# Kiripiro/leaffliction

Hardware: AMD Instinct MI355X
Metric: 224x224 images/sec train (higher is better)
Workload: dtype f32; 1 GPU; leaf_cnn base train step (configs[1]: img 224, batch 256/GPU, fp32, 8 classes, AdamW+clipnorm+EMA, in-model augmentation); per_gpu_batch=256, global_batch=256, img_size=224, parallelism=dp1

## Files before the change

### include/leafhip.h

```cpp
#ifndef LEAFHIP_H
#define LEAFHIP_H

#include <stddef.h>
#include <stdint.h>

#ifdef __cplusplus
extern "C" {
#endif

#define LF_OK 0
#define LF_ERR_INVALID (-1)
#define LF_ERR_LAUNCH (-2)
#define LF_ERR_WORKSPACE (-3)

#define LF_VERSION 100

typedef void* lf_stream_t;

int lf_version(void);
const char* lf_last_error(void);

int lf_copy_rows(void* dst, size_t dst_pitch, const void* src, size_t src_pitch, size_t width, size_t rows, int to_host,
                 lf_stream_t stream);

// ... 211 lines not shown
                                 uint16_t* pooled, int n, int c, int h, int w, lf_stream_t stream);
int lf_block_tail_bwd_bf16(const uint16_t* dp, const uint8_t* route, const uint16_t* y,
                           const float* a_scale, const float* a_shift, const float* drop, uint16_t* dr,
                           float* ds, float* plane_sums, const uint16_t* sc_y, float* sc_sums, int n,
                           int c, int h, int w, lf_stream_t stream);
int lf_bcast_planes_bf16(const float* v, uint16_t* out, int planes, int hw, float scale,
                         lf_stream_t stream);
int lf_cast_f32_bf16(const float* in, uint16_t* out, size_t count, lf_stream_t stream);
int lf_cast_bf16_f32(const uint16_t* in, float* out, size_t count, lf_stream_t stream);

int lf_conv2d_variant(int h, int wd, int cout, int ksize);
int lf_conv2d_wgrad_variant(int n, int cin, int h, int wd, int cout, int ksize);

int lf_conv2d_plan(int n, int cin, int h, int wd, int cout, int ksize, int* out);
int lf_conv2d_wgrad_plan(int n, int cin, int h, int wd, int cout, int ksize, int* out);
int lf_conv2d_bf16_plan(int n, int cin, int h, int w, int cout, int ksize, int x_bf16, int y_bf16, int entry,
                        int accumulate, int mask, int* out);
int lf_conv2d_wgrad_bf16_plan(int n, int cin, int h, int w, int cout, int ksize, int* out);

long long lf_conv2d_stats_tiles(int n, int cin, int h, int w, int cout, int ksize);
int lf_conv2d_stats_f32(const float* x, const float* w, float* y, int n, int cin, int h, int wd,
                        int cout, int ksize, const float* in_scale, const float* in_shift,
                        int in_relu, const float* pivot, float* tile_part, size_t tile_part_bytes,
                        lf_stream_t stream, const float* wino_u);

int lf_conv2d_bnbwd_f32(const float* x, const float* w, float* y, int n, int cin, int h, int wd,
                        int cout, int ksize, int accumulate, const float* mask_y,
                        const float* mask_scale, const float* mask_shift, int mask_relu,
                        float* tile_part, size_t tile_part_bytes, lf_stream_t stream, const float* wino_u);

// ... 98 lines not shown
```

### leaffliction_amd/_lib.py

```python
from __future__ import annotations

import ctypes as C
import os
from pathlib import Path

_LIB = None

LIB_PATH = Path(__file__).resolve().parent / "libleafhip.so"

c_void_p, c_int, c_size_t, c_u64, c_float, c_double = (
    C.c_void_p, C.c_int, C.c_size_t, C.c_uint64, C.c_float, C.c_double)
P = c_void_p

SIGNATURES = {
    "lf_version": [],
    "lf_last_error": [],
    "lf_pack_hwc_u8_to_nchw_f32": [P, P, c_int, c_int, c_int, P, P, P],
    "lf_hist_u8": [P, P, c_int, c_int, c_int, P],
    "lf_autocontrast_lut": [P, P, P, c_int, P],
    "lf_lut_apply_u8": [P, P, P, c_int, c_int, c_int, P],
    "lf_gather_rows_u8": [P, P, P, c_int, c_size_t, P],
    "lf_flip_u8": [P, P, P, c_int, c_int, c_int, P],
    "lf_noise_wrap_add_u8": [P, P, P, c_size_t, P],
    "lf_add_wrap_u8": [P, P, P, c_size_t, P],
# ... 61 lines not shown
    "lf_conv2d_bf16_train": [P, c_int, P, P, c_int, c_int, c_int, c_int, c_int, c_int, P, P, c_int, c_int, P,
                             c_size_t, P, P, P, P, c_int, P],
    "lf_conv2d_wgrad_bf16_workspace": [c_int, c_int, c_int, c_int, c_int, c_int],
    "lf_conv2d_wgrad_bf16": [P, P, P, P, P, P, c_int, P, P, c_int, c_int, c_int, c_int, c_int, c_int, P, P,
                             c_int, P, c_size_t, P],
    "lf_gap_stats_bf16": [P, P, P, c_int, c_int, c_int, P, P, c_int, P],
    "lf_block_tail_fwd_train_bf16": [P, P, P, P, P, P, P, c_int, P, P, P, c_int, c_int, c_int, c_int, P],
    "lf_block_tail_bwd_bf16": [P, P, P, P, P, P, P, P, P, P, P, c_int, c_int, c_int, c_int, P],
    "lf_bcast_planes_bf16": [P, P, c_int, c_int, c_float, P],
    "lf_cast_f32_bf16": [P, P, c_size_t, P],
    "lf_cast_bf16_f32": [P, P, c_size_t, P],
    "lf_conv2d_variant": [c_int, c_int, c_int, c_int],
    "lf_conv2d_wgrad_variant": [c_int, c_int, c_int, c_int, c_int, c_int],
    "lf_conv2d_plan": [c_int, c_int, c_int, c_int, c_int, c_int, P],
    "lf_conv2d_wgrad_plan": [c_int, c_int, c_int, c_int, c_int, c_int, P],
    "lf_conv2d_bf16_plan": [c_int, c_int, c_int, c_int, c_int, c_int, c_int, c_int, c_int, c_int, c_int, P],
    "lf_conv2d_wgrad_bf16_plan": [c_int, c_int, c_int, c_int, c_int, c_int, P],
    "lf_conv2d_stats_tiles": [c_int, c_int, c_int, c_int, c_int, c_int],
    "lf_conv2d_stats_f32": [P, P, P, c_int, c_int, c_int, c_int, c_int, c_int, P, P, c_int, P, P, c_size_t, P, P],
    "lf_conv2d_bnbwd_f32": [P, P, P, c_int, c_int, c_int, c_int, c_int, c_int, c_int, P, P, P, c_int, P,
                            c_size_t, P, P],
    "lf_conv2d_dgrad_weights_f32": [P, P, c_int, c_int, c_int, P],
    "lf_conv2d_takes_wino_filters": [c_int, c_int, c_int, c_int, c_int],
    "lf_conv2d_wino_filters_f32": [P, P, c_int, c_int, c_int, P],
    "lf_conv2d_wgrad_workspace": [c_int, c_int, c_int, c_int, c_int, c_int],
    "lf_conv2d_wgrad_f32": [P, P, c_int, c_int, c_int, c_int, c_int, c_int, P, P, c_int, P,
                            c_size_t, P],
    "lf_conv2d_wgrad_bn_supported": [c_int, c_int, c_int, c_int, c_int, c_int],
    "lf_conv2d_wgrad_bn_f32": [P, P, P, P, P, P, c_int, P, c_int, c_int, c_int, c_int, c_int, c_int, P, P,
                               c_int, P, c_size_t, P],
# ... 78 lines not shown
```

### leaffliction_amd/csrc/lf_conv.hip

```cpp
#include <type_traits>

#include "lf_common.h"

namespace {

typedef float f32x16 __attribute__((ext_vector_type(16)));
typedef float f32x4 __attribute__((ext_vector_type(4)));

constexpr int kThreads = 256;

__device__ __forceinline__ float pro_apply(float v, float sc, float sh, int relu) {
    v = fmaf(v, sc, sh);
    return relu ? fmaxf(v, 0.f) : v;
}

typedef float lf_f4 __attribute__((ext_vector_type(4)));
constexpr unsigned kBufOob = 0xffffffffu;
__device__ __forceinline__ __amdgpu_buffer_rsrc_t buf_rsrc(const float* base, unsigned bytes) {
    return __builtin_amdgcn_make_buffer_rsrc(const_cast<float*>(base), 0, bytes, 0x00020000);
}
__device__ __forceinline__ float4 buf_load4(__amdgpu_buffer_rsrc_t r, unsigned off) {
    const lf_f4 v = __builtin_bit_cast(lf_f4, __builtin_amdgcn_raw_buffer_load_b128(r, off, 0, 0));
    return make_float4(v.x, v.y, v.z, v.w);
}
// ... 2 lines not shown
}

struct ConvArgs {
    const float* x;
    const float* w;
    const float* wino_u;
    float* y;
    const float* in_scale;
    const float* in_shift;
    int n, cin, cout, h, wd;
    int tiles_x, tiles_y;
    int in_relu;
    int accumulate;
    int vec_ok;
    int stack;
    float* stat_part;
    const float* stat_pivot;
    long long stat_tiles;
    const float* stat_mask_y;
    const float* mask_scale;
    const float* mask_shift;
    int mask_relu;
};

using lf::half_sum32;
using lf::row_sum16;

__device__ __forceinline__ void wino_filter(const float (&g)[9], float (&u)[16]) {
    float t[4][3];
#pragma unroll
// ... 41 lines not shown
    for (int r = 0; r < 2; ++r) {
        y[r * 2 + 0] = b[r][0] + b[r][1] + b[r][2];
        y[r * 2 + 1] = b[r][1] - b[r][2] - b[r][3];
    }
}

constexpr int kMaxProC = 512;

template <int TW, int TH, int HALO, bool STK>
struct ConvTile {
    int bz, by, tile;
    int tx0, ty0, n;
    int imgA, gyA0, ra;
    bool imgA_ok, imgB_ok;

    __device__ __forceinline__ explicit ConvTile(const ConvArgs& p) {
        const unsigned gxy = gridDim.x * gridDim.y, gtotal = gxy * gridDim.z;
        const unsigned bflat = blockIdx.x + gridDim.x * (blockIdx.y + gridDim.y * blockIdx.z);
        const unsigned xk = bflat & 7u, xfloor = gtotal >> 3, xrem = gtotal & 7u;
        const unsigned wid_flat = xk * xfloor + (xk < xrem ? xk : xrem) + (bflat >> 3);
        bz = (int)(wid_flat / gxy);
        by = (int)((wid_flat - (unsigned)bz * gxy) / gridDim.x);
        tile = (int)(wid_flat - (unsigned)bz * gxy - (unsigned)by * gridDim.x);
        tx0 = (tile % p.tiles_x) * TW;
        ty0 = (tile / p.tiles_x) * TH;
        n = bz * p.stack;
        imgA = ty0 / p.h;
        gyA0 = ty0 - imgA * p.h;
        ra = min(TH, p.h - gyA0);
        imgA_ok = imgA < p.stack && n + imgA < p.n;
        imgB_ok = STK && imgA + 1 < p.stack && n + imgA + 1 < p.n;
    }

    __device__ __forceinline__ bool patch_row(int py, int h, int& img, int& gy) const {
        if (py < ra + 2 * HALO) {
            img = imgA;
            gy = gyA0 - HALO + py;
            return imgA_ok && gy >= 0 && gy < h;
        }
        img = imgA + 1;
        gy = py - (ra + 2 * HALO) - HALO;
        return imgB_ok && ra < TH && gy >= 0 && gy < h && gy < TH - ra + HALO;
    }
};

template <int TW, int TH, int HALO, bool STK, int kKC>
struct PatchStage {
    static constexpr int PW = TW + 2 * HALO, PH = TH + 2 * HALO + (STK ? 2 * HALO : 0), PP = PW * PH;
    static constexpr int TW4 = TW / 4;
    static constexpr int NVI = kKC * PH * TW4, IPT = (NVI + kThreads - 1) / kThreads;
    static constexpr int NHI = kKC * PH * 2 * HALO, HPT = (NHI + kThreads - 1) / kThreads;
    static_assert(TW % 4 == 0, "float4 patch rows");

    size_t hw;
    float4 pv[IPT];
    float ph[HPT > 0 ? HPT : 1];
    unsigned pg[IPT], pl[IPT];
    unsigned hg[HPT > 0 ? HPT : 1], hl[HPT > 0 ? HPT : 1];
    unsigned okmask = 0;

    __device__ __forceinline__ PatchStage(const ConvArgs& p, const ConvTile<TW, TH, HALO, STK>& t, float* lsc, int tid) {
        if (p.in_scale != nullptr) {
            for (int c = tid; c < p.cin && c < kMaxProC; c += kThreads) {
                lsc[c] = p.in_scale[c];
                lsc[kMaxProC + c] = p.in_shift[c];
            }
        }
        hw = (size_t)p.h * p.wd;
        const unsigned uhw = (unsigned)hw;
#pragma unroll
        for (int i = 0; i < IPT; ++i) {
            const int e = tid + i * kThreads;
            const int kc = e / (PH * TW4), rem = e - kc * (PH * TW4);
            const int py = rem / TW4, slot = rem - py * TW4;
            int img, gy;
            const bool ok = t.patch_row(py, p.h, img, gy) && e < NVI;
            pg[i] = ok ? 4u * ((unsigned)(img * p.cin + kc) * uhw + (unsigned)gy * (unsigned)p.wd + (unsigned)(t.tx0 + 4 * slot)) : kBufOob;
            pl[i] = (unsigned)(kc * PP + py * PW + HALO + 4 * slot) | ((unsigned)kc << 16);
            okmask |= (ok ? 1u : 0u) << i;
        }
#pragma unroll
        for (int i = 0; i < HPT; ++i) {
            const int e = tid + i * kThreads;
            const int kc = e / (PH * 2), rem = e - kc * (PH * 2);
            const int py = rem >> 1, side = rem & 1;
            const int gx = side ? t.tx0 + TW : t.tx0 - 1;
            int img, gy;
            const bool ok = t.patch_row(py, p.h, img, gy) && e < NHI && gx >= 0 && gx < p.wd;
            hg[i] = ok ? 4u * ((unsigned)(img * p.cin + kc) * uhw + (unsigned)gy * (unsigned)p.wd + (unsigned)gx) : kBufOob;
            hl[i] = (unsigned)(kc * PP + py * PW + (side ? PW - 1 : 0)) | ((unsigned)kc << 16);
            okmask |= (ok ? 1u : 0u) << (16 + i);
        }
    }

    __device__ __forceinline__ void load(const ConvArgs& p, const float* xin, int c0) {
        const __amdgpu_buffer_rsrc_t rx = buf_rsrc(
            xin + (size_t)c0 * hw,
            4u * (unsigned)((STK ? (p.stack - 1) * p.cin : 0) + min(kKC, p.cin - c0)) * (unsigned)hw);
#pragma unroll
        for (int i = 0; i < IPT; ++i) pv[i] = buf_load4(rx, pg[i]);
#pragma unroll
        for (int i = 0; i < HPT; ++i) ph[i] = buf_load1(rx, hg[i]);
    }

    __device__ __forceinline__ void store(const ConvArgs& p, float* lp, const float* lsc, int c0, int tid) const {
// ... 144 lines not shown
#pragma unroll
                for (int m = 0; m < MB; ++m)
#pragma unroll
                    for (int nb = 0; nb < NB; ++nb)
                        acc[m][nb] = __builtin_amdgcn_mfma_f32_32x32x2f32(a[m], b[nb], acc[m][nb], 0, 0, 0);
            }
        }
    };

    const int nchunks = (p.cin + kKC - 1) / kKC;
    const bool vec = p.vec_ok && (t.tx0 + TW <= p.wd);

    if (vec) {
        float4 wv[WPT];
        constexpr bool kPrefetchW = MB * NB * 16 <= 64;
        Patch patch(p, t, lsc, tid);
        unsigned wg[WPT];
#pragma unroll
        for (int i = 0; i < WPT; ++i) {
            const int e = tid + i * kThreads;
            const int row = e / CT4, col = (e - row * CT4) * 4;
            wg[i] = (e < NWI && co0 + col < p.cout) ? 4u * ((unsigned)row * (unsigned)p.cout + (unsigned)(co0 + col)) : kBufOob;
        }
        auto load_weights = [&](int c0) {
            const __amdgpu_buffer_rsrc_t rw =
                buf_rsrc(p.w + (size_t)c0 * TAPS * p.cout,
                         4u * (unsigned)(min(kKC, p.cin - c0) * TAPS) * (unsigned)p.cout);
#pragma unroll
            for (int i = 0; i < WPT; ++i) wv[i] = buf_load4(rw, wg[i]);
        };
        auto store_chunk = [&](int c0) {
// ... 110 lines not shown
                        lf::stat_accumulate(acc[m][nb][r], co_ok && pix_ok[nb], true, 0.f, yv[rr][nb], msc, msh,
                                            p.mask_relu, s1, s2);
                }
                s1 = half_sum32(s1);
                s2 = half_sum32(s2);
                if (j == 31) {
                    red[(wave_px * CT + cl) * 2] = s1;
                    red[(wave_px * CT + cl) * 2 + 1] = s2;
                }
            }
        }
    }
    if (stats) write_stat_part<WPX, CT>(p, red, t.bz, t.tile, co0, tid);
}

template <int TW, int TH, int MB, int NB, bool STK>
__global__ __launch_bounds__(kThreads, 2)
void conv_wino_kernel(ConvArgs p) {
    constexpr int kKC = 8, WPX = 4;
    constexpr int TXN = TW / 2, NT = TXN * (TH / 2);
    static_assert(TH % 2 == 0, "F(2x2,3x3): even tile");
    static_assert(WPX * NB * 16 >= NT, "wave decomposition");
    constexpr int CT = 16 * MB;
    constexpr int kUP = 20;
    using Patch = PatchStage<TW, TH, 1, STK, kKC>;
    constexpr int PW = Patch::PW, PP = Patch::PP;
    constexpr int PATCH = kKC * PP;
    constexpr int WSZ = kKC * CT * kUP;
    static_assert(PATCH % 4 == 0, "16-byte aligned U region");

    __shared__ __attribute__((aligned(16))) float lds[PATCH + WSZ];
    __shared__ float lsc[2 * kMaxProC];
    float* lp = lds;
    float* lw = lds + PATCH;

    const int tid = threadIdx.x, lane = tid & 63, wave_px = tid >> 6;
    const ConvTile<TW, TH, 1, STK> t(p);
    const int co0 = t.by * CT;
    const size_t hw = (size_t)p.h * p.wd;
    const unsigned uhw = (unsigned)hw;
    const float* xin = p.x + (size_t)t.n * p.cin * hw;

    const int wq = lane >> 4, wl = lane & 15;
    int vbase[NB];
    const int ubase = (wq * CT + wl) * kUP;
    f32x4 wacc[MB][NB][16];
#pragma unroll
    for (int nb = 0; nb < NB; ++nb) {
        const int tt = min((wave_px * NB + nb) * 16 + wl, NT - 1);
        const int r0 = 2 * (tt / TXN), prow = (STK && r0 >= t.ra) ? r0 + 2 : r0;
        vbase[nb] = wq * PP + prow * PW + 2 * (tt % TXN);
    }
#pragma unroll
    for (int m = 0; m < MB; ++m)
#pragma unroll
        for (int nb = 0; nb < NB; ++nb)
#pragma unroll
            for (int q = 0; q < 16; ++q) wacc[m][nb][q] = f32x4{0.f, 0.f, 0.f, 0.f};

    auto compute_chunk = [&]() {
#pragma unroll
        for (int s = 0; s < kKC / 4; ++s) {
            float u[MB][16];
#pragma unroll
            for (int m = 0; m < MB; ++m) {
                const float4* us = reinterpret_cast<const float4*>(lw + ubase + (4 * s * CT + m * 16) * kUP);
#pragma unroll
                for (int q4 = 0; q4 < 4; ++q4) {
                    const float4 v4 = us[q4];
                    u[m][4 * q4 + 0] = v4.x;
                    u[m][4 * q4 + 1] = v4.y;
                    u[m][4 * q4 + 2] = v4.z;
                    u[m][4 * q4 + 3] = v4.w;
                }
            }
#pragma unroll
            for (int nb = 0; nb < NB; ++nb) {
                const float* src = lp + vbase[nb] + 4 * s * PP;
                float d[16], v[16];
#pragma unroll
                for (int r = 0; r < 4; ++r) {
                    const float2 lo = *reinterpret_cast<const float2*>(src + r * PW);
                    const float2 hi = *reinterpret_cast<const float2*>(src + r * PW + 2);
                    d[r * 4 + 0] = lo.x;
                    d[r * 4 + 1] = lo.y;
                    d[r * 4 + 2] = hi.x;
                    d[r * 4 + 3] = hi.y;
                }
                wino_input(d, v);
#pragma unroll
                for (int m = 0; m < MB; ++m)
#pragma unroll
                    for (int q = 0; q < 16; ++q)
                        wacc[m][nb][q] = __builtin_amdgcn_mfma_f32_16x16x4f32(u[m][q], v[q], wacc[m][nb][q], 0, 0, 0);
            }
        }
    };

    constexpr int KSTEP = kThreads / (4 * CT), UPT = kKC / KSTEP;
    static_assert(kThreads % (4 * CT) == 0 && kKC % KSTEP == 0, "whole channels per pass");
    const int ukc = tid / (4 * CT), uco = (tid >> 2) % CT, uq4 = tid & 3;
    const unsigned ustep = 64u * KSTEP * (unsigned)p.cout;
    const unsigned ugo = co0 + uco < p.cout ? 4u * (((unsigned)ukc * (unsigned)p.cout + (unsigned)(co0 + uco)) * 16u + 4u * (unsigned)uq4) : 0x80000000u;
    float* const ulds = lw + (ukc * CT + uco) * kUP + 4 * uq4;
    float4 uv[UPT];
    auto load_u = [&](int c0) {
        const __amdgpu_buffer_rsrc_t ru =
            buf_rsrc(p.wino_u + (size_t)c0 * p.cout * 16, 64u * (unsigned)min(kKC, p.cin - c0) * (unsigned)p.cout);
#pragma unroll
        for (int i = 0; i < UPT; ++i) uv[i] = buf_load4(ru, ugo + (unsigned)i * ustep);
    };
    auto store_u = [&]() {
#pragma unroll
        for (int i = 0; i < UPT; ++i) *reinterpret_cast<float4*>(ulds + i * KSTEP * CT * kUP) = uv[i];
    };

    const int nchunks = (p.cin + kKC - 1) / kKC;
    const bool vec = p.vec_ok && (t.tx0 + TW <= p.wd);

    if (vec) {
        Patch patch(p, t, lsc, tid);
        patch.load(p, xin, 0);
        for (int ch = 0; ch < nchunks; ++ch) {
            __syncthreads();
            load_u(ch * kKC);
            patch.store(p, lp, lsc, ch * kKC, tid);
            store_u();
            __syncthreads();
            if (ch + 1 < nchunks) patch.load(p, xin, (ch + 1) * kKC);
            compute_chunk();
        }
    } else {
        for (int ch = 0; ch < nchunks; ++ch) {
            const int c0 = ch * kKC;
            __syncthreads();
            Patch::stage_scalar(p, lp, xin, t.tx0, t.ty0, c0, tid);
            load_u(c0);
            store_u();
            __syncthreads();
            compute_chunk();
        }
    }

    float* yout = p.y + (size_t)t.n * p.cout * hw;
    const bool stats = p.stat_part != nullptr, masked = p.stat_mask_y != nullptr;
    float* red = lds;
    static_assert(WPX * CT * 2 <= PATCH + WSZ, "stat scratch must fit the staging LDS");
    if (stats) __syncthreads();
    const float* my = masked ? p.stat_mask_y + (size_t)t.n * p.cout * hw : nullptr;
    const bool y2 = (p.wd & 1) == 0 && (reinterpret_cast<size_t>(p.y) & 7) == 0;
    bool pok[NB][4];
    unsigned pofs[NB][4];
#pragma unroll
    for (int nb = 0; nb < NB; ++nb) {
        const int tt = (wave_px * NB + nb) * 16 + wl;
        const int r0 = 2 * (tt / TXN), ox = t.tx0 + 2 * (tt % TXN);
        const bool in_a = r0 < t.ra;
        const int oy = in_a ? t.gyA0 + r0 : r0 - t.ra;
        const bool img_ok = tt < NT && (in_a ? t.imgA_ok : t.imgB_ok);
        const unsigned base = (unsigned)((in_a ? t.imgA : t.imgA + 1) * p.cout) * uhw;
#pragma unroll
        for (int q = 0; q < 4; ++q) {
            const int py = oy + (q >> 1), px = ox + (q & 1);
            pok[nb][q] = img_ok && py < p.h && px < p.wd;
            pofs[nb][q] = pok[nb][q] ? base + (unsigned)py * (unsigned)p.wd + (unsigned)px : 0u;
        }
    }
#pragma unroll
    for (int m = 0; m < MB; ++m) {
#pragma unroll
        for (int i = 0; i < 4; ++i) {
            const int cl = m * 16 + 4 * wq + i;
            const int co = co0 + cl;
            const bool co_ok = co < p.cout;
            const size_t cofs = (size_t)min(co, p.cout - 1) * hw;
            float out[NB][4], oldv[NB][4], yv[NB][4];
#pragma unroll
            for (int nb = 0; nb < NB; ++nb) {
                float mm[16];
#pragma unroll
                for (int q = 0; q < 16; ++q) mm[q] = wacc[m][nb][q][i];
                wino_output(mm, out[nb]);
                if (p.accumulate) {
#pragma unroll
                    for (int q = 0; q < 4; ++q) oldv[nb][q] = yout[cofs + pofs[nb][q]];
                }
                if (masked) {
#pragma unroll
                    for (int q = 0; q < 4; ++q) yv[nb][q] = my[cofs + pofs[nb][q]];
                }
            }
#pragma unroll
            for (int nb = 0; nb < NB; ++nb) {
                if (p.accumulate) {
#pragma unroll
                    for (int q = 0; q < 4; ++q) out[nb][q] += oldv[nb][q];
                }
                if (co_ok) {
#pragma unroll
                    for (int r = 0; r < 2; ++r) {
                        float* dst = yout + cofs + pofs[nb][2 * r];
                        if (y2 && pok[nb][2 * r] && pok[nb][2 * r + 1]) {
                            *reinterpret_cast<float2*>(dst) = make_float2(out[nb][2 * r], out[nb][2 * r + 1]);
                        } else {
                            if (pok[nb][2 * r]) dst[0] = out[nb][2 * r];
                            if (pok[nb][2 * r + 1]) yout[cofs + pofs[nb][2 * r + 1]] = out[nb][2 * r + 1];
                        }
                    }
                }
            }
            if (!stats) continue;
            float s1 = 0.f, s2 = 0.f;
            if (!masked) {
                const float pv = (p.stat_pivot != nullptr && co_ok) ? p.stat_pivot[co] : 0.f;
#pragma unroll
                for (int nb = 0; nb < NB; ++nb)
#pragma unroll
                    for (int q = 0; q < 4; ++q)
                        lf::stat_accumulate(out[nb][q], pok[nb][q], false, pv, 0.f, 0.f, 0.f, 0, s1, s2);
            } else {
                const float msc = p.mask_scale[min(co, p.cout - 1)], msh = p.mask_shift[min(co, p.cout - 1)];
#pragma unroll
                for (int nb = 0; nb < NB; ++nb)
#pragma unroll
                    for (int q = 0; q < 4; ++q)
                        lf::stat_accumulate(out[nb][q], co_ok && pok[nb][q], true, 0.f, yv[nb][q], msc, msh, p.mask_relu,
                                            s1, s2);
            }
            s1 = row_sum16(s1);
            s2 = row_sum16(s2);
            if (wl == 0) {
                red[(wave_px * CT + cl) * 2] = s1;
                red[(wave_px * CT + cl) * 2 + 1] = s2;
            }
        }
    }
    if (stats) write_stat_part<WPX, CT>(p, red, t.bz, t.tile, co0, tid);
}

struct WgradArgs {
    const float* x;
    const float* dy;
    float* part;
    const float* in_scale;
    const float* in_shift;
    int n, cin, cout, h, wd;
    int tiles_x, tiles_y, items, items_per_split;
    int in_relu;
    int vec_ok;
    const float* bn_y;
    const float* bn_alpha;
    const float* bn_add;
// ... 848 lines not shown
};
constexpr FwdVariant kFwdVariants[] = {{32, 8, 32}, {32, 8, 64}, {16, 16, 32}, {16, 16, 64},
                                       {28, 8, 128}, {32, 8, 128}, {56, 8, 64}};
constexpr int kNumFwd = sizeof(kFwdVariants) / sizeof(kFwdVariants[0]);

inline long long padded_work(const FwdVariant& v, int h, int w, int cout) {
    const long long tx = (w + v.tw - 1) / v.tw, ty = (h + v.th - 1) / v.th,
                    tc = (cout + v.ct - 1) / v.ct;
    return tx * v.tw * ty * v.th * tc * v.ct;
}

inline bool fwd_small_cin(int taps, int variant, int cin) { return taps == 9 && variant == 0 && cin <= 4; }

inline bool fwd_vec_shape(int wd, int cout) { return wd % 4 == 0 && cout % 4 == 0; }

int launch_fwd(int ksize, int variant, const ConvArgs& a, unsigned gx, unsigned gz, hipStream_t s) {
    const auto grid = [&](int ct) { return dim3(gx, (a.cout + ct - 1) / ct, gz); };
    const dim3 g = grid(kFwdVariants[variant].ct);
    if (ksize == 3 && fwd_small_cin(9, variant, a.cin)) {
        conv_mfma_kernel<9, 32, 8, 1, 1, 4, 2, 4><<<g, kThreads, 0, s>>>(a);
        return LF_OK;
    }
    if (ksize == 3) {
        switch (variant) {
            case 0: conv_wino_kernel<32, 8, 2, 1, false><<<grid(32), kThreads, 0, s>>>(a); break;
            case 2: conv_wino_kernel<16, 16, 2, 1, false><<<grid(32), kThreads, 0, s>>>(a); break;
            case 4: conv_wino_kernel<28, 8, 2, 1, true><<<grid(32), kThreads, 0, s>>>(a); break;
            case 6: conv_wino_kernel<56, 8, 1, 2, false><<<grid(16), kThreads, 0, s>>>(a); break;
            default: return LF_ERR_INVALID;
        }
        return LF_OK;
    }
    switch (variant) {
        case 0: conv_mfma_kernel<1, 32, 8, 1, 1, 4, 2, 8><<<g, kThreads, 0, s>>>(a); break;
        case 1: conv_mfma_kernel<1, 32, 8, 1, 2, 4, 2, 8><<<g, kThreads, 0, s>>>(a); break;
        case 2: conv_mfma_kernel<1, 16, 16, 1, 1, 4, 2, 8><<<g, kThreads, 0, s>>>(a); break;
        case 3: conv_mfma_kernel<1, 16, 16, 1, 2, 4, 2, 8><<<g, kThreads, 0, s>>>(a); break;
        case 4: conv_mfma_kernel<1, 28, 8, 4, 1, 1, 7, 8, true><<<g, kThreads, 0, s>>>(a); break;
        case 5: conv_mfma_kernel<1, 32, 8, 2, 2, 2, 4, 8><<<g, kThreads, 0, s>>>(a); break;
        case 6: conv_mfma_kernel<1, 56, 8, 2, 1, 2, 7, 8><<<g, kThreads, 0, s>>>(a); break;
        default: return LF_ERR_INVALID;
    }
    return LF_OK;
}

struct WgVariant {
// ... 252 lines not shown
    return conv2d_launch("lf_conv2d_bnbwd", x, w, wino_u, y, n, cin, h, wd, cout, ksize, nullptr, nullptr, 0,
                         accumulate, tile_part, nullptr, mask_y, mask_scale, mask_shift, mask_relu,
                         stream);
}

int lf_conv2d_dgrad_weights_f32(const float* w, float* wt, int cin, int ksize, int cout,
                                lf_stream_t stream) {
    LF_REQUIRE(w && wt, "lf_conv2d_dgrad_weights: null buffer");
    LF_REQUIRE(cin > 0 && cout > 0 && (ksize == 1 || ksize == 3), "lf_conv2d_dgrad_weights: bad dims");
    const int total = cin * ksize * ksize * cout;
    weight_dgrad_kernel<<<lf::stream_grid(total, kThreads), kThreads, 0, lf::as_stream(stream)>>>(
        w, wt, cin, ksize * ksize, cout);
    return lf::check_launch("lf_conv2d_dgrad_weights");
}

int lf_conv2d_takes_wino_filters(int cin, int h, int wd, int cout, int ksize) {
    if (cin <= 0 || cout <= 0 || h <= 0 || wd <= 0) return 0;
    return fwd_takes_wino_filters(cin, h, wd, cout, ksize) ? 1 : 0;
}

int lf_conv2d_wino_filters_f32(const float* w, float* u, int cin, int cout, int dgrad, lf_stream_t stream) {
    LF_REQUIRE(w && u, "lf_conv2d_wino_filters: null buffer");
    LF_REQUIRE(cin > 0 && cout > 0 && (size_t)cin * cout * 16 < (1ull << 30), "lf_conv2d_wino_filters: bad dims");
    LF_REQUIRE(aligned16(u), "lf_conv2d_wino_filters: u must be 16-byte aligned");
    wino_filters_kernel<<<lf::stream_grid((size_t)cin * cout, kThreads), kThreads, 0, lf::as_stream(stream)>>>(
        w, u, cin, cout, dgrad ? 1 : 0);
    return lf::check_launch("lf_conv2d_wino_filters");
}

size_t lf_conv2d_wgrad_workspace(int n, int cin, int h, int wd, int cout, int ksize) {
// ... 92 lines not shown
```

### leaffliction_amd/nn.py

```python
from __future__ import annotations

import os
from typing import Optional

import torch

from . import _lib
from .ops import _chk, _stream

_F32 = torch.float32
_BF16 = torch.bfloat16
_ws_cache = {}
_ws_gen = 0
_NO_FUSED_BN_WGRAD = os.environ.get("LEAFFLICTION_NO_FUSED_BN_WGRAD", "0") == "1"


def _workspace(nbytes: int, device, slot: int = 0) -> torch.Tensor:
    global _ws_gen
    key = (str(device), slot)
    buf = _ws_cache.get(key)
    if buf is None or buf.numel() < nbytes:
        if torch.cuda.is_available() and torch.cuda.is_current_stream_capturing():
            raise RuntimeError("a workspace would have to grow while a HIP graph is being recorded: run the shape "
                               "eagerly first (the warm-up steps size every workspace)")
# ... 1 lines not shown
        _ws_cache[key] = buf
        _ws_gen += 1
    return buf


def workspace_generation() -> int:
    return _ws_gen


def _ptr(t: Optional[torch.Tensor]):
    return None if t is None else t.data_ptr()


def conv2d_takes_wino_filters(cin: int, h: int, w: int, cout: int, ksize: int) -> bool:
    return bool(_lib.load().lf_conv2d_takes_wino_filters(int(cin), int(h), int(w), int(cout), int(ksize)))


def conv2d_wino_filters(w_iko: torch.Tensor, dgrad: bool = False,
                        out: Optional[torch.Tensor] = None) -> torch.Tensor:
    _chk(w_iko, _F32, "conv2d_wino_filters.w", 3)
    cin, taps, cout = w_iko.shape
    if taps != 9:
        raise ValueError("conv2d_wino_filters: 3x3 weights [Cin,9,Cout] expected")
    shape = (cout, cin, 16) if dgrad else (cin, cout, 16)
    if out is None:
        out = torch.empty(shape, dtype=_F32, device=w_iko.device)
    else:
        _chk(out, _F32, "conv2d_wino_filters.out", 3)
        if tuple(out.shape) != shape:
            raise ValueError(f"conv2d_wino_filters.out: expected {shape}")
# ... 587 lines not shown
```

Baseline: 6215 images/sec.

## Make Winograd 3x3 conv kernel persistent with prefetch of next tile

Converts the Winograd forward conv kernel into a persistent kernel that launches about twice as many blocks as CUs and walks work items in a loop. Where PRE is set it prefetches the next tile's patch while finishing the current one. The goal is to cut block launch and tail overhead and to overlap global loads across tiles. In exchange it adds register pressure, a CU-count query that cannot run during graph capture on first use, and a tunable cap.

```diff
diff --git a/include/leafhip.h b/include/leafhip.h
--- a/include/leafhip.h
+++ b/include/leafhip.h
@@ -249,6 +249,7 @@
 
 int lf_conv2d_plan(int n, int cin, int h, int wd, int cout, int ksize, int* out);
 int lf_conv2d_wgrad_plan(int n, int cin, int h, int wd, int cout, int ksize, int* out);
+int lf_conv2d_wino_set_cap(int cap);
 int lf_conv2d_bf16_plan(int n, int cin, int h, int w, int cout, int ksize, int x_bf16, int y_bf16, int entry,
                         int accumulate, int mask, int* out);
 int lf_conv2d_wgrad_bf16_plan(int n, int cin, int h, int w, int cout, int ksize, int* out);
diff --git a/leaffliction_amd/_lib.py b/leaffliction_amd/_lib.py
--- a/leaffliction_amd/_lib.py
+++ b/leaffliction_amd/_lib.py
@@ -99,6 +99,7 @@
     "lf_conv2d_wgrad_variant": [c_int, c_int, c_int, c_int, c_int, c_int],
     "lf_conv2d_plan": [c_int, c_int, c_int, c_int, c_int, c_int, P],
     "lf_conv2d_wgrad_plan": [c_int, c_int, c_int, c_int, c_int, c_int, P],
+    "lf_conv2d_wino_set_cap": [c_int],
     "lf_conv2d_bf16_plan": [c_int, c_int, c_int, c_int, c_int, c_int, c_int, c_int, c_int, c_int, c_int, P],
     "lf_conv2d_wgrad_bf16_plan": [c_int, c_int, c_int, c_int, c_int, c_int, P],
     "lf_conv2d_stats_tiles": [c_int, c_int, c_int, c_int, c_int, c_int],
diff --git a/leaffliction_amd/csrc/lf_conv.hip b/leaffliction_amd/csrc/lf_conv.hip
--- a/leaffliction_amd/csrc/lf_conv.hip
+++ b/leaffliction_amd/csrc/lf_conv.hip
@@ -1,3 +1,4 @@
+#include <atomic>
 #include <type_traits>
 
 #include "lf_common.h"
@@ -40,6 +41,7 @@
     int accumulate;
     int vec_ok;
     int stack;
+    unsigned items_x, items_y, items_z;
     float* stat_part;
     const float* stat_pivot;
     long long stat_tiles;
@@ -111,14 +113,11 @@
     int imgA, gyA0, ra;
     bool imgA_ok, imgB_ok;
 
-    __device__ __forceinline__ explicit ConvTile(const ConvArgs& p) {
-        const unsigned gxy = gridDim.x * gridDim.y, gtotal = gxy * gridDim.z;
-        const unsigned bflat = blockIdx.x + gridDim.x * (blockIdx.y + gridDim.y * blockIdx.z);
-        const unsigned xk = bflat & 7u, xfloor = gtotal >> 3, xrem = gtotal & 7u;
-        const unsigned wid_flat = xk * xfloor + (xk < xrem ? xk : xrem) + (bflat >> 3);
-        bz = (int)(wid_flat / gxy);
-        by = (int)((wid_flat - (unsigned)bz * gxy) / gridDim.x);
-        tile = (int)(wid_flat - (unsigned)bz * gxy - (unsigned)by * gridDim.x);
+    __device__ __forceinline__ ConvTile(const ConvArgs& p, unsigned item, unsigned gx, unsigned gy) {
+        const unsigned gxy = gx * gy;
+        bz = (int)(item / gxy);
+        by = (int)((item - (unsigned)bz * gxy) / gx);
+        tile = (int)(item - (unsigned)bz * gxy - (unsigned)by * gx);
         tx0 = (tile % p.tiles_x) * TW;
         ty0 = (tile / p.tiles_x) * TH;
         n = bz * p.stack;
@@ -129,6 +128,16 @@
         imgB_ok = STK && imgA + 1 < p.stack && n + imgA + 1 < p.n;
     }
 
+    __device__ __forceinline__ explicit ConvTile(const ConvArgs& p)
+        : ConvTile(p, grid_item(), gridDim.x, gridDim.y) {}
+
+    static __device__ __forceinline__ unsigned grid_item() {
+        const unsigned gtotal = gridDim.x * gridDim.y * gridDim.z;
+        const unsigned bflat = blockIdx.x + gridDim.x * (blockIdx.y + gridDim.y * blockIdx.z);
+        const unsigned xk = bflat & 7u, xfloor = gtotal >> 3, xrem = gtotal & 7u;
+        return xk * xfloor + (xk < xrem ? xk : xrem) + (bflat >> 3);
+    }
+
     __device__ __forceinline__ bool patch_row(int py, int h, int& img, int& gy) const {
         if (py < ra + 2 * HALO) {
             img = imgA;
@@ -138,6 +147,19 @@
         img = imgA + 1;
         gy = py - (ra + 2 * HALO) - HALO;
         return imgB_ok && ra < TH && gy >= 0 && gy < h && gy < TH - ra + HALO;
+    }
+};
+
+struct ItemWalk {
+    unsigned it, end, step;
+    __device__ __forceinline__ explicit ItemWalk(unsigned items) {
+        const unsigned g = gridDim.x, b = blockIdx.x;
+        const unsigned nx = g < 8u ? g : 8u;
+        const unsigned xk = b % nx, sfloor = items / nx, srem = items % nx;
+        const unsigned first = xk * sfloor + (xk < srem ? xk : srem);
+        step = g / nx + (xk < g % nx ? 1u : 0u);
+        it = first + b / nx;
+        end = first + sfloor + (xk < srem ? 1u : 0u);
     }
 };
 
@@ -156,7 +178,7 @@
     unsigned hg[HPT > 0 ? HPT : 1], hl[HPT > 0 ? HPT : 1];
     unsigned okmask = 0;
 
-    __device__ __forceinline__ PatchStage(const ConvArgs& p, const ConvTile<TW, TH, HALO, STK>& t, float* lsc, int tid) {
+    __device__ __forceinline__ PatchStage(const ConvArgs& p, float* lsc, int tid) {
         if (p.in_scale != nullptr) {
             for (int c = tid; c < p.cin && c < kMaxProC; c += kThreads) {
                 lsc[c] = p.in_scale[c];
@@ -164,7 +186,29 @@
             }
         }
         hw = (size_t)p.h * p.wd;
+        place(tid);
+    }
+
+    __device__ __forceinline__ void place(int tid) {
+#pragma unroll
+        for (int i = 0; i < IPT; ++i) {
+            const int e = tid + i * kThreads;
+            const int kc = e / (PH * TW4), rem = e - kc * (PH * TW4);
+            const int py = rem / TW4, slot = rem - py * TW4;
+            pl[i] = (unsigned)(kc * PP + py * PW + HALO + 4 * slot) | ((unsigned)kc << 16);
+        }
+#pragma unroll
+        for (int i = 0; i < HPT; ++i) {
+            const int e = tid + i * kThreads;
+            const int kc = e / (PH * 2), rem = e - kc * (PH * 2);
+            const int py = rem >> 1, side = rem & 1;
+            hl[i] = (unsigned)(kc * PP + py * PW + (side ? PW - 1 : 0)) | ((unsigned)kc << 16);
+        }
+    }
+
+    __device__ __forceinline__ void aim(const ConvArgs& p, const ConvTile<TW, TH, HALO, STK>& t, int tid) {
         const unsigned uhw = (unsigned)hw;
+        okmask = 0;
 #pragma unroll
         for (int i = 0; i < IPT; ++i) {
             const int e = tid + i * kThreads;
@@ -173,7 +217,6 @@
             int img, gy;
             const bool ok = t.patch_row(py, p.h, img, gy) && e < NVI;
             pg[i] = ok ? 4u * ((unsigned)(img * p.cin + kc) * uhw + (unsigned)gy * (unsigned)p.wd + (unsigned)(t.tx0 + 4 * slot)) : kBufOob;
-            pl[i] = (unsigned)(kc * PP + py * PW + HALO + 4 * slot) | ((unsigned)kc << 16);
             okmask |= (ok ? 1u : 0u) << i;
         }
 #pragma unroll
@@ -185,7 +228,6 @@
             int img, gy;
             const bool ok = t.patch_row(py, p.h, img, gy) && e < NHI && gx >= 0 && gx < p.wd;
             hg[i] = ok ? 4u * ((unsigned)(img * p.cin + kc) * uhw + (unsigned)gy * (unsigned)p.wd + (unsigned)gx) : kBufOob;
-            hl[i] = (unsigned)(kc * PP + py * PW + (side ? PW - 1 : 0)) | ((unsigned)kc << 16);
             okmask |= (ok ? 1u : 0u) << (16 + i);
         }
     }
@@ -360,7 +402,8 @@
     if (vec) {
         float4 wv[WPT];
         constexpr bool kPrefetchW = MB * NB * 16 <= 64;
-        Patch patch(p, t, lsc, tid);
+        Patch patch(p, lsc, tid);
+        patch.aim(p, t, tid);
         unsigned wg[WPT];
 #pragma unroll
         for (int i = 0; i < WPT; ++i) {
@@ -501,7 +544,12 @@
     if (stats) write_stat_part<WPX, CT>(p, red, t.bz, t.tile, co0, tid);
 }
 
-template <int TW, int TH, int MB, int NB, bool STK>
+__device__ __forceinline__ int here(int v) {
+    asm volatile("" : "+v"(v));
+    return v;
+}
+
+template <int TW, int TH, int MB, int NB, bool STK, bool PRE>
 __global__ __launch_bounds__(kThreads, 2)
 void conv_wino_kernel(ConvArgs p) {
     constexpr int kKC = 8, WPX = 4;
@@ -510,6 +558,7 @@
     static_assert(WPX * NB * 16 >= NT, "wave decomposition");
     constexpr int CT = 16 * MB;
     constexpr int kUP = 20;
+    using Tile = ConvTile<TW, TH, 1, STK>;
     using Patch = PatchStage<TW, TH, 1, STK, kKC>;
     constexpr int PW = Patch::PW, PP = Patch::PP;
     constexpr int PATCH = kKC * PP;
@@ -521,208 +570,244 @@
     float* lp = lds;
     float* lw = lds + PATCH;
 
-    const int tid = threadIdx.x, lane = tid & 63, wave_px = tid >> 6;
-    const ConvTile<TW, TH, 1, STK> t(p);
-    const int co0 = t.by * CT;
     const size_t hw = (size_t)p.h * p.wd;
     const unsigned uhw = (unsigned)hw;
-    const float* xin = p.x + (size_t)t.n * p.cin * hw;
-
-    const int wq = lane >> 4, wl = lane & 15;
-    int vbase[NB];
-    const int ubase = (wq * CT + wl) * kUP;
-    f32x4 wacc[MB][NB][16];
-#pragma unroll
-    for (int nb = 0; nb < NB; ++nb) {
-        const int tt = min((wave_px * NB + nb) * 16 + wl, NT - 1);
-        const int r0 = 2 * (tt / TXN), prow = (STK && r0 >= t.ra) ? r0 + 2 : r0;
-        vbase[nb] = wq * PP + prow * PW + 2 * (tt % TXN);
-    }
-#pragma unroll
-    for (int m = 0; m < MB; ++m)
-#pragma unroll
-        for (int nb = 0; nb < NB; ++nb)
-#pragma unroll
-            for (int q = 0; q < 16; ++q) wacc[m][nb][q] = f32x4{0.f, 0.f, 0.f, 0.f};
-
-    auto compute_chunk = [&]() {
-#pragma unroll
-        for (int s = 0; s < kKC / 4; ++s) {
-            float u[MB][16];
-#pragma unroll
-            for (int m = 0; m < MB; ++m) {
-                const float4* us = reinterpret_cast<const float4*>(lw + ubase + (4 * s * CT + m * 16) * kUP);
-#pragma unroll
-                for (int q4 = 0; q4 < 4; ++q4) {
-                    const float4 v4 = us[q4];
-                    u[m][4 * q4 + 0] = v4.x;
-                    u[m][4 * q4 + 1] = v4.y;
-                    u[m][4 * q4 + 2] = v4.z;
-                    u[m][4 * q4 + 3] = v4.w;
-                }
-            }
-#pragma unroll
-            for (int nb = 0; nb < NB; ++nb) {
-                const float* src = lp + vbase[nb] + 4 * s * PP;
-                float d[16], v[16];
-#pragma unroll
-                for (int r = 0; r < 4; ++r) {
-                    const float2 lo = *reinterpret_cast<const float2*>(src + r * PW);
-                    const float2 hi = *reinterpret_cast<const float2*>(src + r * PW + 2);
-                    d[r * 4 + 0] = lo.x;
-                    d[r * 4 + 1] = lo.y;
-                    d[r * 4 + 2] = hi.x;
-                    d[r * 4 + 3] = hi.y;
-                }
-                wino_input(d, v);
-#pragma unroll
-                for (int m = 0; m < MB; ++m)
-#pragma unroll
-                    for (int q = 0; q < 16; ++q)
-                        wacc[m][nb][q] = __builtin_amdgcn_mfma_f32_16x16x4f32(u[m][q], v[q], wacc[m][nb][q], 0, 0, 0);
-            }
-        }
-    };
-
-    constexpr int KSTEP = kThreads / (4 * CT), UPT = kKC / KSTEP;
-    static_assert(kThreads % (4 * CT) == 0 && kKC % KSTEP == 0, "whole channels per pass");
-    const int ukc = tid / (4 * CT), uco = (tid >> 2) % CT, uq4 = tid & 3;
-    const unsigned ustep = 64u * KSTEP * (unsigned)p.cout;
-    const unsigned ugo = co0 + uco < p.cout ? 4u * (((unsigned)ukc * (unsigned)p.cout + (unsigned)(co0 + uco)) * 16u + 4u * (unsigned)uq4) : 0x80000000u;
-    float* const ulds = lw + (ukc * CT + uco) * kUP + 4 * uq4;
-    float4 uv[UPT];
-    auto load_u = [&](int c0) {
-        const __amdgpu_buffer_rsrc_t ru =
-            buf_rsrc(p.wino_u + (size_t)c0 * p.cout * 16, 64u * (unsigned)min(kKC, p.cin - c0) * (unsigned)p.cout);
-#pragma unroll
-        for (int i = 0; i < UPT; ++i) uv[i] = buf_load4(ru, ugo + (unsigned)i * ustep);
-    };
-    auto store_u = [&]() {
-#pragma unroll
-        for (int i = 0; i < UPT; ++i) *reinterpret_cast<float4*>(ulds + i * KSTEP * CT * kUP) = uv[i];
-    };
-
     const int nchunks = (p.cin + kKC - 1) / kKC;
-    const bool vec = p.vec_ok && (t.tx0 + TW <= p.wd);
-
-    if (vec) {
-        Patch patch(p, t, lsc, tid);
-        patch.load(p, xin, 0);
-        for (int ch = 0; ch < nchunks; ++ch) {
-            __syncthreads();
-            load_u(ch * kKC);
-            patch.store(p, lp, lsc, ch * kKC, tid);
-            store_u();
-            __syncthreads();
-            if (ch + 1 < nchunks) patch.load(p, xin, (ch + 1) * kKC);
-            compute_chunk();
-        }
-    } else {
-        for (int ch = 0; ch < nchunks; ++ch) {
-            const int c0 = ch * kKC;
-            __syncthreads();
-            Patch::stage_scalar(p, lp, xin, t.tx0, t.ty0, c0, tid);
-            load_u(c0);
-            store_u();
-            __syncthreads();
-            compute_chunk();
-        }
-    }
-
-    float* yout = p.y + (size_t)t.n * p.cout * hw;
     const bool stats = p.stat_part != nullptr, masked = p.stat_mask_y != nullptr;
     float* red = lds;
     static_assert(WPX * CT * 2 <= PATCH + WSZ, "stat scratch must fit the staging LDS");
-    if (stats) __syncthreads();
-    const float* my = masked ? p.stat_mask_y + (size_t)t.n * p.cout * hw : nullptr;
     const bool y2 = (p.wd & 1) == 0 && (reinterpret_cast<size_t>(p.y) & 7) == 0;
-    bool pok[NB][4];
-    unsigned pofs[NB][4];
-#pragma unroll
-    for (int nb = 0; nb < NB; ++nb) {
-        const int tt = (wave_px * NB + nb) * 16 + wl;
-        const int r0 = 2 * (tt / TXN), ox = t.tx0 + 2 * (tt % TXN);
-        const bool in_a = r0 < t.ra;
-        const int oy = in_a ? t.gyA0 + r0 : r0 - t.ra;
-        const bool img_ok = tt < NT && (in_a ? t.imgA_ok : t.imgB_ok);
-        const unsigned base = (unsigned)((in_a ? t.imgA : t.imgA + 1) * p.cout) * uhw;
-#pragma unroll
-        for (int q = 0; q < 4; ++q) {
-            const int py = oy + (q >> 1), px = ox + (q & 1);
-            pok[nb][q] = img_ok && py < p.h && px < p.wd;
-            pofs[nb][q] = pok[nb][q] ? base + (unsigned)py * (unsigned)p.wd + (unsigned)px : 0u;
-        }
-    }
-#pragma unroll
-    for (int m = 0; m < MB; ++m) {
-#pragma unroll
-        for (int i = 0; i < 4; ++i) {
-            const int cl = m * 16 + 4 * wq + i;
-            const int co = co0 + cl;
-            const bool co_ok = co < p.cout;
-            const size_t cofs = (size_t)min(co, p.cout - 1) * hw;
-            float out[NB][4], oldv[NB][4], yv[NB][4];
-#pragma unroll
-            for (int nb = 0; nb < NB; ++nb) {
-                float mm[16];
-#pragma unroll
-                for (int q = 0; q < 16; ++q) mm[q] = wacc[m][nb][q][i];
-                wino_output(mm, out[nb]);
-                if (p.accumulate) {
-#pragma unroll
-                    for (int q = 0; q < 4; ++q) oldv[nb][q] = yout[cofs + pofs[nb][q]];
-                }
-                if (masked) {
-#pragma unroll
-                    for (int q = 0; q < 4; ++q) yv[nb][q] = my[cofs + pofs[nb][q]];
-                }
-            }
-#pragma unroll
-            for (int nb = 0; nb < NB; ++nb) {
-                if (p.accumulate) {
-#pragma unroll
-                    for (int q = 0; q < 4; ++q) out[nb][q] += oldv[nb][q];
-                }
-                if (co_ok) {
-#pragma unroll
-                    for (int r = 0; r < 2; ++r) {
-                        float* dst = yout + cofs + pofs[nb][2 * r];
-                        if (y2 && pok[nb][2 * r] && pok[nb][2 * r + 1]) {
-                            *reinterpret_cast<float2*>(dst) = make_float2(out[nb][2 * r], out[nb][2 * r + 1]);
-                        } else {
-                            if (pok[nb][2 * r]) dst[0] = out[nb][2 * r];
-                            if (pok[nb][2 * r + 1]) yout[cofs + pofs[nb][2 * r + 1]] = out[nb][2 * r + 1];
+    const bool m2 = y2 && (reinterpret_cast<size_t>(p.stat_mask_y) & 7) == 0;
+
+    Patch patch(p, lsc, threadIdx.x);
+    ItemWalk walk(p.items_x * p.items_y * p.items_z);
+    Tile t(p, walk.it, p.items_x, p.items_y);
+    bool vec = p.vec_ok && (t.tx0 + TW <= p.wd);
+    bool aimed = false;
+    for (;;) {
+        const int tid = here(threadIdx.x), lane = tid & 63, wave_px = tid >> 6;
+        const int co0 = t.by * CT;
+        const float* xin = p.x + (size_t)t.n * p.cin * hw;
+        patch.place(tid);
+
+        const int wq = lane >> 4, wl = lane & 15;
+        const int ubase = (wq * CT + wl) * kUP;
+        int vbase[NB];
+    #pragma unroll
+        for (int nb = 0; nb < NB; ++nb) {
+            const int tt = min((wave_px * NB + nb) * 16 + wl, NT - 1);
+            const int r0 = 2 * (tt / TXN), prow = (STK && r0 >= t.ra) ? r0 + 2 : r0;
+            vbase[nb] = wq * PP + prow * PW + 2 * (tt % TXN);
+        }
+        f32x4 wacc[MB][NB][16];
+
+        auto compute_chunk = [&]() {
+    #pragma unroll
+            for (int s = 0; s < kKC / 4; ++s) {
+                float u[MB][16];
+    #pragma unroll
+                for (int m = 0; m < MB; ++m) {
+                    const float4* us = reinterpret_cast<const float4*>(lw + ubase + (4 * s * CT + m * 16) * kUP);
+    #pragma unroll
+                    for (int q4 = 0; q4 < 4; ++q4) {
+                        const float4 v4 = us[q4];
+                        u[m][4 * q4 + 0] = v4.x;
+                        u[m][4 * q4 + 1] = v4.y;
+                        u[m][4 * q4 + 2] = v4.z;
+                        u[m][4 * q4 + 3] = v4.w;
+                    }
+                }
+    #pragma unroll
+                for (int nb = 0; nb < NB; ++nb) {
+                    const float* src = lp + vbase[nb] + 4 * s * PP;
+                    float d[16], v[16];
+    #pragma unroll
+                    for (int r = 0; r < 4; ++r) {
+                        const float2 lo = *reinterpret_cast<const float2*>(src + r * PW);
+                        const float2 hi = *reinterpret_cast<const float2*>(src + r * PW + 2);
+                        d[r * 4 + 0] = lo.x;
+                        d[r * 4 + 1] = lo.y;
+                        d[r * 4 + 2] = hi.x;
+                        d[r * 4 + 3] = hi.y;
+                    }
+                    wino_input(d, v);
+    #pragma unroll
+                    for (int m = 0; m < MB; ++m)
+    #pragma unroll
+                        for (int q = 0; q < 16; ++q)
+                            wacc[m][nb][q] = __builtin_amdgcn_mfma_f32_16x16x4f32(u[m][q], v[q], wacc[m][nb][q], 0, 0, 0);
+                }
+            }
+        };
+
+        constexpr int KSTEP = kThreads / (4 * CT), UPT = kKC / KSTEP;
+        static_assert(kThreads % (4 * CT) == 0 && kKC % KSTEP == 0, "whole channels per pass");
+        const int ukc = tid / (4 * CT), uco = (tid >> 2) % CT, uq4 = tid & 3;
+        const unsigned ustep = 64u * KSTEP * (unsigned)p.cout;
+        const unsigned ugo = co0 + uco < p.cout ? 4u * (((unsigned)ukc * (unsigned)p.cout + (unsigned)(co0 + uco)) * 16u + 4u * (unsigned)uq4) : 0x80000000u;
+        float* const ulds = lw + (ukc * CT + uco) * kUP + 4 * uq4;
+        float4 uv[UPT];
+        auto load_u = [&](int c0) {
+            const __amdgpu_buffer_rsrc_t ru =
+                buf_rsrc(p.wino_u + (size_t)c0 * p.cout * 16, 64u * (unsigned)min(kKC, p.cin - c0) * (unsigned)p.cout);
+    #pragma unroll
+            for (int i = 0; i < UPT; ++i) uv[i] = buf_load4(ru, ugo + (unsigned)i * ustep);
+        };
+        auto store_u = [&]() {
+    #pragma unroll
+            for (int i = 0; i < UPT; ++i) *reinterpret_cast<float4*>(ulds + i * KSTEP * CT * kUP) = uv[i];
+        };
+
+#pragma unroll
+        for (int m = 0; m < MB; ++m)
+#pragma unroll
+            for (int nb = 0; nb < NB; ++nb)
+#pragma unroll
+                for (int q = 0; q < 16; ++q) wacc[m][nb][q] = f32x4{0.f, 0.f, 0.f, 0.f};
+
+        const unsigned nit = walk.it + walk.step;
+        const bool more = nit < walk.end;
+        bool pre = false;
+
+        if (vec) {
+            if (!aimed) {
+                patch.aim(p, t, tid);
+                patch.load(p, xin, 0);
+            }
+            for (int ch = 0; ch < nchunks; ++ch) {
+                __syncthreads();
+                load_u(ch * kKC);
+                patch.store(p, lp, lsc, ch * kKC, tid);
+                store_u();
+                __syncthreads();
+                if (ch + 1 < nchunks) {
+                    patch.load(p, xin, (ch + 1) * kKC);
+                } else if (PRE && more) {
+                    const Tile tn(p, nit, p.items_x, p.items_y);
+                    if (tn.tx0 + TW <= p.wd) {
+                        patch.aim(p, tn, tid);
+                        patch.load(p, p.x + (size_t)tn.n * p.cin * hw, 0);
+                        pre = true;
+                    }
+                }
+                compute_chunk();
+            }
+        } else {
+            for (int ch = 0; ch < nchunks; ++ch) {
+                const int c0 = ch * kKC;
+                __syncthreads();
+                Patch::stage_scalar(p, lp, xin, t.tx0, t.ty0, c0, tid);
+                load_u(c0);
+                store_u();
+                __syncthreads();
+                compute_chunk();
+            }
+        }
+
+        float* yout = p.y + (size_t)t.n * p.cout * hw;
+        if (stats) __syncthreads();
+        const float* my = masked ? p.stat_mask_y + (size_t)t.n * p.cout * hw : nullptr;
+        bool pok[NB][4];
+        unsigned pofs[NB][4];
+#pragma unroll
+        for (int nb = 0; nb < NB; ++nb) {
+            const int tt = (wave_px * NB + nb) * 16 + wl;
+            const int r0 = 2 * (tt / TXN), ox = t.tx0 + 2 * (tt % TXN);
+            const bool in_a = r0 < t.ra;
+            const int oy = in_a ? t.gyA0 + r0 : r0 - t.ra;
+            const bool img_ok = tt < NT && (in_a ? t.imgA_ok : t.imgB_ok);
+            const unsigned base = (unsigned)((in_a ? t.imgA : t.imgA + 1) * p.cout) * uhw;
+#pragma unroll
+            for (int q = 0; q < 4; ++q) {
+                const int py = oy + (q >> 1), px = ox + (q & 1);
+                pok[nb][q] = img_ok && py < p.h && px < p.wd;
+                pofs[nb][q] = pok[nb][q] ? base + (unsigned)py * (unsigned)p.wd + (unsigned)px : 0u;
+            }
+        }
+        auto load4 = [&](const float* src, const unsigned (&ofs)[4], bool pairs, float (&v)[4]) {
+            if (pairs) {
+#pragma unroll
+                for (int r = 0; r < 2; ++r) {
+                    const float2 v2 = *reinterpret_cast<const float2*>(src + ofs[2 * r]);
+                    v[2 * r] = v2.x;
+                    v[2 * r + 1] = v2.y;
+                }
+            } else {
+#pragma unroll
+                for (int q = 0; q < 4; ++q) v[q] = src[ofs[q]];
+            }
+        };
+#pragma unroll
+        for (int m = 0; m < MB; ++m) {
+#pragma unroll
+            for (int i = 0; i < 4; ++i) {
+                const int cl = m * 16 + 4 * wq + i;
+                const int co = co0 + cl;
+                const bool co_ok = co < p.cout;
+                const size_t cofs = (size_t)min(co, p.cout - 1) * hw;
+                float out[NB][4], oldv[NB][4], yv[NB][4];
+#pragma unroll
+                for (int nb = 0; nb < NB; ++nb) {
+                    float mm[16];
+#pragma unroll
+                    for (int q = 0; q < 16; ++q) mm[q] = wacc[m][nb][q][i];
+                    wino_output(mm, out[nb]);
+                    if (p.accumulate) load4(yout + cofs, pofs[nb], y2, oldv[nb]);
+                    if (masked) load4(my + cofs, pofs[nb], m2, yv[nb]);
+                }
+#pragma unroll
+                for (int nb = 0; nb < NB; ++nb) {
+                    if (p.accumulate) {
+#pragma unroll
+                        for (int q = 0; q < 4; ++q) out[nb][q] += oldv[nb][q];
+                    }
+                    if (co_ok) {
+#pragma unroll
+                        for (int r = 0; r < 2; ++r) {
+                            float* dst = yout + cofs + pofs[nb][2 * r];
+                            if (y2 && pok[nb][2 * r] && pok[nb][2 * r + 1]) {
+                                *reinterpret_cast<float2*>(dst) = make_float2(out[nb][2 * r], out[nb][2 * r + 1]);
+                            } else {
+                                if (pok[nb][2 * r]) dst[0] = out[nb][2 * r];
+                                if (pok[nb][2 * r + 1]) yout[cofs + pofs[nb][2 * r + 1]] = out[nb][2 * r + 1];
+                            }
                         }
                     }
                 }
-            }
-            if (!stats) continue;
-            float s1 = 0.f, s2 = 0.f;
-            if (!masked) {
-                const float pv = (p.stat_pivot != nullptr && co_ok) ? p.stat_pivot[co] : 0.f;
-#pragma unroll
-                for (int nb = 0; nb < NB; ++nb)
-#pragma unroll
-                    for (int q = 0; q < 4; ++q)
-                        lf::stat_accumulate(out[nb][q], pok[nb][q], false, pv, 0.f, 0.f, 0.f, 0, s1, s2);
-            } else {
-                const float msc = p.mask_scale[min(co, p.cout - 1)], msh = p.mask_shift[min(co, p.cout - 1)];
-#pragma unroll
-                for (int nb = 0; nb < NB; ++nb)
-#pragma unroll
-                    for (int q = 0; q < 4; ++q)
-                        lf::stat_accumulate(out[nb][q], co_ok && pok[nb][q], true, 0.f, yv[nb][q], msc, msh, p.mask_relu,
-                                            s1, s2);
-            }
-            s1 = row_sum16(s1);
-            s2 = row_sum16(s2);
-            if (wl == 0) {
-                red[(wave_px * CT + cl) * 2] = s1;
-                red[(wave_px * CT + cl) * 2 + 1] = s2;
-            }
-        }
-    }
-    if (stats) write_stat_part<WPX, CT>(p, red, t.bz, t.tile, co0, tid);
+                if (!stats) continue;
+                float s1 = 0.f, s2 = 0.f;
+                if (!masked) {
+                    const float pv = (p.stat_pivot != nullptr && co_ok) ? p.stat_pivot[co] : 0.f;
+#pragma unroll
+                    for (int nb = 0; nb < NB; ++nb)
+#pragma unroll
+                        for (int q = 0; q < 4; ++q)
+                            lf::stat_accumulate(out[nb][q], pok[nb][q], false, pv, 0.f, 0.f, 0.f, 0, s1, s2);
+                } else {
+                    const float msc = p.mask_scale[min(co, p.cout - 1)], msh = p.mask_shift[min(co, p.cout - 1)];
+#pragma unroll
+                    for (int nb = 0; nb < NB; ++nb)
+#pragma unroll
+                        for (int q = 0; q < 4; ++q)
+                            lf::stat_accumulate(out[nb][q], co_ok && pok[nb][q], true, 0.f, yv[nb][q], msc, msh, p.mask_relu,
+                                                s1, s2);
+                }
+                s1 = row_sum16(s1);
+                s2 = row_sum16(s2);
+                if (wl == 0) {
+                    red[(wave_px * CT + cl) * 2] = s1;
+                    red[(wave_px * CT + cl) * 2 + 1] = s2;
+                }
+            }
+        }
+        if (stats) write_stat_part<WPX, CT>(p, red, t.bz, t.tile, co0, tid);
+
+        if (!more) break;
+        t = Tile(p, nit, p.items_x, p.items_y);
+        vec = p.vec_ok && (t.tx0 + TW <= p.wd);
+        aimed = pre;
+        walk.it = nit;
+    }
 }
 
 struct WgradArgs {
@@ -1601,22 +1686,64 @@
 
 inline bool fwd_vec_shape(int wd, int cout) { return wd % 4 == 0 && cout % 4 == 0; }
 
+std::atomic<int> g_wino_cap{0};
+constexpr int kMaxDevices = 64;
+std::atomic<int> g_cu_count[kMaxDevices];
+
+int device_cu_count(hipStream_t s) {
+    int dev = 0;
+    if (hipGetDevice(&dev) != hipSuccess || dev < 0 || dev >= kMaxDevices) {
+        lf::set_error("conv2d: no current device");
+        return 0;
+    }
+    int cus = g_cu_count[dev].load(std::memory_order_relaxed);
+    if (cus > 0) return cus;
+    hipStreamCaptureStatus st = hipStreamCaptureStatusNone;
+    if (hipStreamIsCapturing(s, &st) != hipSuccess || st != hipStreamCaptureStatusNone) {
+        lf::set_error("conv2d: the first 3x3 launch on a device asks for its CU count and cannot be captured into a graph");
+        return 0;
+    }
+    if (hipDeviceGetAttribute(&cus, hipDeviceAttributeMultiprocessorCount, dev) != hipSuccess || cus <= 0) {
+        lf::set_error("conv2d: cannot read the device's CU count");
+        return 0;
+    }
+    g_cu_count[dev].store(cus, std::memory_order_relaxed);
+    return cus;
+}
+
 int launch_fwd(int ksize, int variant, const ConvArgs& a, unsigned gx, unsigned gz, hipStream_t s) {
-    const auto grid = [&](int ct) { return dim3(gx, (a.cout + ct - 1) / ct, gz); };
-    const dim3 g = grid(kFwdVariants[variant].ct);
+    const dim3 g(gx, (a.cout + kFwdVariants[variant].ct - 1) / kFwdVariants[variant].ct, gz);
     if (ksize == 3 && fwd_small_cin(9, variant, a.cin)) {
         conv_mfma_kernel<9, 32, 8, 1, 1, 4, 2, 4><<<g, kThreads, 0, s>>>(a);
         return LF_OK;
     }
     if (ksize == 3) {
+        const auto launch = [&](auto kernel, int ct) {
+            ConvArgs w = a;
+            w.items_x = gx;
+            w.items_y = (unsigned)((a.cout + ct - 1) / ct);
+            w.items_z = gz;
+            const unsigned long long items = (unsigned long long)w.items_x * w.items_y * w.items_z;
+            if (items >= (1ull << 32)) {
+                lf::set_error("conv2d: %llu work items do not fit 32 bits", items);
+                return LF_ERR_INVALID;
+            }
+            int cap = g_wino_cap.load(std::memory_order_relaxed);
+            if (cap <= 0) {
+                const int cus = device_cu_count(s);
+                if (cus <= 0) return LF_ERR_LAUNCH;
+                cap = 2 * cus;
+            }
+            kernel<<<dim3((unsigned)(items < (unsigned long long)cap ? items : (unsigned long long)cap)), kThreads, 0, s>>>(w);
+            return LF_OK;
+        };
         switch (variant) {
-            case 0: conv_wino_kernel<32, 8, 2, 1, false><<<grid(32), kThreads, 0, s>>>(a); break;
-            case 2: conv_wino_kernel<16, 16, 2, 1, false><<<grid(32), kThreads, 0, s>>>(a); break;
-            case 4: conv_wino_kernel<28, 8, 2, 1, true><<<grid(32), kThreads, 0, s>>>(a); break;
-            case 6: conv_wino_kernel<56, 8, 1, 2, false><<<grid(16), kThreads, 0, s>>>(a); break;
+            case 0: return launch(conv_wino_kernel<32, 8, 2, 1, false, true>, 32);
+            case 2: return launch(conv_wino_kernel<16, 16, 2, 1, false, true>, 32);
+            case 4: return launch(conv_wino_kernel<28, 8, 2, 1, true, true>, 32);
+            case 6: return launch(conv_wino_kernel<56, 8, 1, 2, false, false>, 16);
             default: return LF_ERR_INVALID;
         }
-        return LF_OK;
     }
     switch (variant) {
         case 0: conv_mfma_kernel<1, 32, 8, 1, 1, 4, 2, 8><<<g, kThreads, 0, s>>>(a); break;
@@ -1899,6 +2026,11 @@
     return lf::check_launch("lf_conv2d_dgrad_weights");
 }
 
+int lf_conv2d_wino_set_cap(int cap) {
+    g_wino_cap.store(cap > 0 ? cap : 0, std::memory_order_relaxed);
+    return LF_OK;
+}
+
 int lf_conv2d_takes_wino_filters(int cin, int h, int wd, int cout, int ksize) {
     if (cin <= 0 || cout <= 0 || h <= 0 || wd <= 0) return 0;
     return fwd_takes_wino_filters(cin, h, wd, cout, ksize) ? 1 : 0;
diff --git a/leaffliction_amd/nn.py b/leaffliction_amd/nn.py
--- a/leaffliction_amd/nn.py
+++ b/leaffliction_amd/nn.py
@@ -1,5 +1,6 @@
 from __future__ import annotations
 
+import ctypes
 import os
 from typing import Optional
 
@@ -39,6 +40,16 @@
 
 def conv2d_takes_wino_filters(cin: int, h: int, w: int, cout: int, ksize: int) -> bool:
     return bool(_lib.load().lf_conv2d_takes_wino_filters(int(cin), int(h), int(w), int(cout), int(ksize)))
+
+
+def conv2d_plan(n: int, cin: int, h: int, w: int, cout: int, ksize: int):
+    out = (ctypes.c_int * 4)()
+    _lib.call("lf_conv2d_plan", int(n), int(cin), int(h), int(w), int(cout), int(ksize), out)
+    return tuple(out)
+
+
+def conv2d_wino_set_cap(cap: int = 0) -> None:
+    _lib.call("lf_conv2d_wino_set_cap", int(cap))
 
 
 def conv2d_wino_filters(w_iko: torch.Tensor, dgrad: bool = False,
```

New measurement: 5924 images/sec. 4.7% lower.
